# kowallus/mbgc

Measured on AMD Instinct MI355X. Metric: input Gbases/s (compress hot path, -m1: match-finding + stream emission), higher is better.
Workload: dtype u8

## Files before the change

mbgc_amd/csrc/swsem_emit.hip:

```cpp
#include "swsem_device.h"
#include "../../include/mbgc_swsem.h"

namespace swk {

constexpr int EMIT_THREADS = 1024;
constexpr uint8_t MATCH_MARK = 0xA5;
constexpr int MAX_EXTEND_MATCH_LEFT_LENGTH = 1 << 24;

struct EMatch {
    uint64_t posSrc, len, posDest, lp;
};

struct EmitContig {
    uint64_t qoff, n;
    uint64_t matchBase;
    uint64_t lock;
    uint64_t scratchBase;
    uint64_t streamBase[SWSEM_NSTREAMS];
    uint32_t cap;
    uint32_t chunk0;
    int32_t factor;
    uint32_t span0;
    int64_t processed, targetIdx;
};

struct EmitOut {
    uint64_t size[SWSEM_NSTREAMS];
    uint64_t unmatchedChars;
    uint64_t extMatched, extMismatches, totalMatched, removed, nmatches;
};

struct LongCopy { uint8_t *dst; const uint8_t *src; uint64_t len; };
constexpr uint32_t LONG_COPY_CAP = 4096;
constexpr uint32_t LONG_COPY_MIN = 32768;

struct EmitView {
    const uint8_t *ref, *qbuf;
    const Match *matches;
    const uint32_t *matchCount;
    uint64_t pos1, refLength, maxRefLength;
    const uint64_t *loaded; uint32_t nLoaded;
    swsem_emit_params_t p;
    EMatch *em;
    uint64_t *next0;
    uint8_t *removed;
    uint32_t *keepIdx;
    uint32_t *meta;
    uint32_t *corr;
    unsigned long long *pairMask;
    unsigned long long *litBits;
    unsigned long long *metaBad;
    uint32_t *sz;
    uint32_t *ofs;
    uint32_t *chunkCnt;
    const uint32_t *chunkOwner;
    const uint32_t *spanOwner;
    uint32_t ncontigs;
    uint64_t *packBase;
    uint8_t *arena;
    struct LongCopy *longCopies;
    uint32_t *longCount;
    EmitOut *out;
};

constexpr uint32_t META_SKIPOFF = 1, META_HASGAP = 2, META_ISGAP = 4, META_GSTART = 8, META_GMID = 16, META_GEND = 32;

__device__ __forceinline__ bool paired(uint64_t aSrc, uint64_t aDst, uint64_t bSrc, uint64_t bDst) {
    return aSrc + bDst == bSrc + aDst;
}

__device__ __forceinline__ int sym5(uint8_t c) {
    return c == 'A' ? 0 : c == 'C' ? 1 : c == 'G' ? 2 : c == 'T' ? 3 : c == 'N' ? 4 : -1;
}
__device__ __forceinline__ uint8_t mismatch2code(uint8_t actual, uint8_t mismatch) {
    const int a = sym5(actual), b = sym5(mismatch);
    if (actual == mismatch || a < 0 || b < 0) return mismatch;
    const uint32_t rows[5] = {0 | 2u << 3 | 0u << 6 | 1u << 9 | 3u << 12, 1 | 0u << 3 | 2u << 6 | 0u << 9 | 3u << 12,
                              0 | 2u << 3 | 0u << 6 | 1u << 9 | 3u << 12, 1 | 0u << 3 | 2u << 6 | 0u << 9 | 3u << 12,
                              1 | 2u << 3 | 3u << 6 | 0u << 9 | 0u << 12};
    return (uint8_t) ((rows[a] >> (3 * b)) & 7u);
}

__device__ __forceinline__ uint64_t loaded_pos(const EmitView &v, uint64_t pos) {
    const uint64_t span = v.refLength - 1;
    const uint64_t back = v.loaded[v.nLoaded - 1];
    while (pos + span < back) pos += span;
    return pos;
}

template <int NT>
__device__ uint32_t block_scan(uint32_t x, uint32_t *lds, uint32_t *total) {
    const uint32_t lane = threadIdx.x & (WAVE - 1), w = threadIdx.x / WAVE;
    uint32_t inc = x;
    for (int d = 1; d < WAVE; d <<= 1) {
        const uint32_t y = (uint32_t) __shfl_up((int) inc, d);
        if ((int) lane >= d) inc += y;
    }
    __syncthreads();
    if (lane == WAVE - 1) lds[w] = inc;
    __syncthreads();
    if (threadIdx.x == 0) {
        uint32_t run = 0;
        for (int i = 0; i < NT / WAVE; i++) { const uint32_t t = lds[i]; lds[i] = run; run += t; }
        lds[NT / WAVE] = run;
    }
    __syncthreads();
    *total = lds[NT / WAVE];
    return lds[w] + inc - x;
}

constexpr int CH = 256;

__device__ __forceinline__ bool p1_flag(const EmitView &v, const Match *__restrict__ M, int64_t n, int64_t j) {
    if (!v.p.enableExtensionsWithMismatches || j < 1 || j + 1 >= n) return false;
    const Match a = M[j - 1], b = M[j], c = M[j + 1];
    return paired(c.posSrc, c.posDest, a.posSrc, a.posDest) && !paired(b.posSrc, b.posDest, a.posSrc, a.posDest) &&
           b.len < v.p.gapBreakingMatchMinLength;
}

__global__ void __launch_bounds__(CH) k_emit_p1_removed(EmitView v, const EmitContig *__restrict__ cgs, const int *__restrict__ which) {
    __shared__ uint32_t cnt;
    const uint32_t gk = v.chunkOwner[blockIdx.x];
    const EmitContig cg = cgs[gk];
    const uint32_t gx = blockIdx.x - cg.chunk0;
    const int64_t n = v.matchCount[which[gk]];
    if ((int64_t) gx * CH >= n) { if (threadIdx.x == 0) v.chunkCnt[(size_t) blockIdx.x] = 0; return; }
    const int64_t j = (int64_t) gx * CH + threadIdx.x;
    if (threadIdx.x == 0) cnt = 0;
    __syncthreads();
    const Match *M = v.matches + cg.matchBase;
    bool keep = false;
    if (j < n) {
        bool r = false;
// ... 241 lines not shown
                st.claimed |= 1ull << (gf - 1);
                if (lazy) {
                    const int t = k + gf;
                    if (t < WAVE) st.nxA = wl64(nextj, t, st.nxA);
                    else st.nxB = wl64(nextj, t - WAVE, st.nxB);
                }
                if (ext && st.gapEndIdx <= j + gf && gf <= v.p.gapDepthMismatchesEncoding) { st.gapStartIdx = j; st.gapEndIdx = j + gf; }
            }
            st.curClaimed = st.claimed & 1ull;
            st.claimed >>= 1;
            if (WRITE) {
                const bool gs = st.gapStartIdx == j, ge = st.gapEndIdx == j + 1, gm = st.gapStartIdx < j && j + 1 < st.gapEndIdx;
                const bool isGap = gs || gm || ge;
                const uint32_t mw = (skipOffset ? META_SKIPOFF : 0) | (gCnt ? META_HASGAP : 0) | (isGap ? META_ISGAP : 0) |
                                    (gs ? META_GSTART : 0) | (gm ? META_GMID : 0) | (ge ? META_GEND : 0) | (gapByte << 8);
                metaV = wl32(mw, k, metaV);
                corrV = wl32(isGap ? (uint32_t) st.gapStartIdx : (uint32_t) j, k, corrV);
            }
        }
        if (WRITE && lane < cnt) {
            v.meta[cg.scratchBase + jl] = metaV;
            v.corr[cg.scratchBase + jl] = corrV;
        }
        st.nxA = st.nxB;
        st.nxB = 0;
    }
}


__device__ __forceinline__ bool mrec_equal(const MetaRec &a, const MetaRec &b) {
    uint32_t ra, rb;
    __builtin_memcpy(&ra, a.rel, 4); __builtin_memcpy(&rb, b.rel, 4);
    uint64_t d = (a.claimed ^ b.claimed) | (uint64_t) (a.gapStartIdx ^ b.gapStartIdx) | (uint64_t) (a.gapEndIdx ^ b.gapEndIdx) |
                 (uint64_t) (a.flags ^ b.flags) | (uint64_t) (ra ^ rb);
#pragma unroll
    for (int e = 0; e < MNX; e++) d |= a.val[e] ^ b.val[e];
    return d == 0;
}

__device__ __forceinline__ void mrec_store(MetaRec *dst, unsigned long long claimed, bool cur, int gs, int ge, const int (&nxPos)[MNX],
                                           const uint64_t (&nxVal)[MNX], bool overflow, int J) {
    uint32_t r[MNX]; uint64_t x[MNX];
#pragma unroll
    for (int e = 0; e < MNX; e++) { r[e] = nxPos[e] >= J ? (uint32_t) (nxPos[e] - J) : 0xFFu; x[e] = nxPos[e] >= J ? nxVal[e] : 0; }
    auto cx = [&](int a, int b) {
        if (r[a] > r[b]) { const uint32_t t = r[a]; r[a] = r[b]; r[b] = t; const uint64_t u = x[a]; x[a] = x[b]; x[b] = u; }
    };
    cx(0, 1); cx(2, 3); cx(0, 2); cx(1, 3); cx(1, 2);
    MetaRec R;
    R.claimed = claimed; R.gapStartIdx = gs; R.gapEndIdx = ge;
    R.flags = (cur ? MREC_CUR : 0u) | (overflow ? MREC_OVERFLOW : 0u);
#pragma unroll
    for (int e = 0; e < MNX; e++) { R.rel[e] = (uint8_t) r[e]; R.val[e] = x[e]; }
    *dst = R;
}

struct MetaSpan { uint32_t gk; int n, B0; bool live; };
__device__ __forceinline__ MetaSpan meta_span(const EmitView &v, const EmitContig *__restrict__ cgs) {
    MetaSpan sp;
    sp.gk = v.spanOwner[blockIdx.x];
    const EmitOut o = v.out[sp.gk];
    sp.n = (int) o.nmatches;
    sp.B0 = (int) (blockIdx.x - cgs[sp.gk].span0) * MSPAN;
    sp.live = o.unmatchedChars != UINT64_MAX && sp.B0 < sp.n;
    return sp;
}

__global__ void __launch_bounds__(CH) k_emit_meta_regions(EmitView v, const EmitContig *__restrict__ cgs) {
    if (!v.p.lazyDecompressionSupport) return;
    const uint32_t gk = v.chunkOwner[blockIdx.x];
    const EmitContig cg = cgs[gk];
    const uint32_t gx = blockIdx.x - cg.chunk0;
    const EmitOut o = v.out[gk];
    if (o.unmatchedChars == UINT64_MAX) return;
    const uint64_t t = (uint64_t) gx * CH + threadIdx.x;
    if (t >= o.nmatches) return;
    const uint64_t lp = loaded_pos(v, v.em[cg.scratchBase + t].posSrc);
    v.em[cg.scratchBase + t].lp = lp;
    uint32_t lo = 0, hi = v.nLoaded;
    while (lo < hi) { const uint32_t mid = (lo + hi) / 2; if (v.loaded[mid] <= lp) lo = mid + 1; else hi = mid; }
    v.next0[cg.scratchBase + t] = lo == v.nLoaded ? UINT64_MAX : v.loaded[lo];
}

__global__ void __launch_bounds__(MLANES) k_emit_meta_masks(EmitView v, const EmitContig *__restrict__ cgs) {
    __shared__ uint64_t skey[MPAD_SIZE], slp[MPAD_SIZE];
    const MetaSpan sp = meta_span(v, cgs);
    if (!sp.live) return;
    const EmitContig cg = cgs[sp.gk];
    const int n = sp.n, B0 = sp.B0, tid = (int) threadIdx.x;
    const int P1 = B0 + MSPAN < n ? B0 + MSPAN : n;
    const int PK = P1 + WAVE < n ? P1 + WAVE : n;
    const EMatch *E = v.em + cg.scratchBase;
    const bool lazy = v.p.lazyDecompressionSupport != 0;
    const int depth = v.p.gapDepthOffsetEncoding;
    for (int i = tid; i < ((PK - B0 + WAVE - 1) & ~(WAVE - 1)); i += MLANES) {
        const int m = B0 + i;
        bool lit0 = false;
        if (m < PK) {
            const EMatch e = E[m];
            const uint64_t side = e.posSrc > cg.lock ? 1u : (e.posSrc < cg.lock ? 2u : 0u);
            skey[mpad(i)] = ((e.posSrc - e.posDest) << 2) | side;
            slp[mpad(i)] = e.lp;
            const uint64_t nxt = m + 1 < n ? E[m + 1].posDest : cg.n;
            lit0 = nxt - (uint32_t) (e.posDest + e.len) == 0;
        }
        const unsigned long long lb = __ballot(lit0);
        if ((tid & (WAVE - 1)) == 0 && m < P1) v.litBits[(size_t) cg.chunk0 * (CH / WAVE) + (size_t) (m / WAVE)] = lb;
    }
    __syncthreads();
    for (int i = tid; i < P1 - B0; i += MLANES) {
        const int m = B0 + i;
        const int gCnt = n - m - 1 < depth ? n - m - 1 : depth;
        const uint64_t kj = skey[mpad(i)];
        const uint64_t own = lazy ? v.next0[cg.scratchBase + m] : UINT64_MAX;
        unsigned long long pm = 0;
#pragma unroll 8
        for (int g = 1; g <= WAVE; g++) {
            const int x = mpad(g <= gCnt ? i + g : i);
            const bool ok = (g <= gCnt) & (skey[x] == kj) & ((slp[x] < own) | !lazy);
            pm |= (unsigned long long) ok << (g - 1);
        }
        v.pairMask[cg.scratchBase + m] = pm;
    }
}

__global__ void __launch_bounds__(MLANES) k_emit_meta_spec(EmitView v, const EmitContig *__restrict__ cgs, MetaRec *__restrict__ recs, int warm,
                                                          unsigned long long *__restrict__ stats) {
    __shared__ uint64_t spm[MPAD_SIZE], sown[MPAD_SIZE];
    __shared__ unsigned long long slit[MPAD_N / WAVE + 2];
    const MetaSpan sp = meta_span(v, cgs);
    if (!sp.live) return;
    const EmitContig cg = cgs[sp.gk];
    const int n = sp.n, B0 = sp.B0, tid = (int) threadIdx.x;
    const int P0 = B0 >= MWARM ? B0 - MWARM : 0;
    const int P1 = B0 + MSPAN < n ? B0 + MSPAN : n;
    const EMatch *E = v.em + cg.scratchBase;
    const bool lazy = v.p.lazyDecompressionSupport != 0, ext = v.p.enableExtensionsWithMismatches != 0;
    const int depth = v.p.gapDepthOffsetEncoding, depthMism = v.p.gapDepthMismatchesEncoding;
    const int PK = P1 + WAVE < n ? P1 + WAVE : n;
    for (int i = tid; i < PK - P0; i += MLANES) {
        if (P0 + i < P1) spm[mpad(i)] = v.pairMask[cg.scratchBase + P0 + i];
        sown[mpad(i)] = lazy ? v.next0[cg.scratchBase + P0 + i] : 0;
    }
    if (tid < MPAD_N / WAVE + 2) {
        const int w = P0 / WAVE + tid;
        slit[tid] = w * WAVE < P1 ? v.litBits[(size_t) cg.chunk0 * (CH / WAVE) + (size_t) w] : 0;
    }
    __syncthreads();
    const int j0 = B0 + tid * MB;
    const bool active = j0 < n;
    const int j1 = j0 + MB < n ? j0 + MB : n;
    unsigned long long claimed = 0;
    bool cur = false, overflow = false;
    int gs = -1, ge = -1;
    int nxPos[MNX]; uint64_t nxVal[MNX];
#pragma unroll
    for (int e = 0; e < MNX; e++) { nxPos[e] = -1; nxVal[e] = 0; }
    MetaRec *myRecs = recs + ((size_t) cg.chunk0 * (CH / MB) + (size_t) (j0 / MB)) * 2;
    for (int s = 0; s < MWARM + MB; s++) {
        const int j = j0 - MWARM + s;
        if (s == MWARM && active) mrec_store(myRecs, claimed, cur, gs, ge, nxPos, nxVal, overflow, j0);
        if (!active || j < j0 - warm || j < 0 || j >= j1) continue;
        const int i = j - P0;
        if (ext && j == ge) { gs = -1; ge = -1; }
        const bool skipOffset = cur;
        const int gCnt = n - j - 1 < depth ? n - j - 1 : depth;
        const bool rule = !lazy && gs == -1 && ((slit[i / WAVE] >> (i & (WAVE - 1))) & 1);
        const unsigned long long taken = claimed | (rule ? 1ull : 0ull);
        unsigned long long em = spm[mpad(i)] & ~taken;
        uint64_t inherited = 0;
#pragma unroll
        for (int e = 0; e < MNX; e++) if (nxPos[e] == j) { inherited = nxVal[e]; nxPos[e] = -1; }
        uint64_t nextj = 0;
        if (lazy) {
            nextj = sown[mpad(i)];
            if (inherited && inherited != nextj) {
                nextj = inherited;
                atomicAdd(&stats[4], 1ull);
                const EMatch mj = E[j];
                em = 0;
                for (int g = 1; g <= gCnt; g++) {
                    const EMatch c = E[j + g];
                    const bool pw = paired(mj.posSrc, mj.posDest, c.posSrc, c.posDest) &&
                                    ((mj.posSrc > cg.lock && c.posSrc > cg.lock) || (mj.posSrc < cg.lock && c.posSrc < cg.lock));
                    if (pw && c.lp < nextj) em |= 1ull << (g - 1);
                }
                em &= ~taken;
            }
        }
        uint32_t gapByte = 0;
        if (em) {
            const int gf = __builtin_ctzll(em) + 1;
            const unsigned long long below = gf > 1 ? ((1ull << (gf - 1)) - 1) : 0ull;
            gapByte = (uint32_t) (gf - __popcll(taken & below));
            claimed |= 1ull << (gf - 1);
            if (lazy && nextj != sown[mpad(i + gf)]) {
                bool put = false;
#pragma unroll
                for (int e = 0; e < MNX; e++) if (!put && nxPos[e] < 0) { nxPos[e] = j + gf; nxVal[e] = nextj; put = true; }
                overflow |= !put;
            }
            if (ext && ge <= j + gf && gf <= depthMism) { gs = j; ge = j + gf; }
        }
        cur = claimed & 1ull;
        claimed >>= 1;
        if (j >= j0) {
            const bool s0 = gs == j, e0 = ge == j + 1, m0 = gs < j && j + 1 < ge;
            const bool isGap = s0 || m0 || e0;
            const uint32_t mw = (skipOffset ? META_SKIPOFF : 0) | (gCnt ? META_HASGAP : 0) | (isGap ? META_ISGAP : 0) |
                                (s0 ? META_GSTART : 0) | (m0 ? META_GMID : 0) | (e0 ? META_GEND : 0) | (gapByte << 8);
            v.meta[cg.scratchBase + j] = mw;
            v.corr[cg.scratchBase + j] = (uint32_t) (isGap ? gs : j);
        }
    }
    if (active) mrec_store(myRecs + 1, claimed, cur, gs, ge, nxPos, nxVal, overflow, j1);
    if (active && overflow) atomicAdd(&stats[7], 1ull);
}

__global__ void __launch_bounds__(WAVE) k_emit_meta_check(EmitView v, const EmitContig *__restrict__ cgs, const MetaRec *__restrict__ recs,
                                                          unsigned long long *__restrict__ stats) {
    constexpr int CPW = WAVE * MB / CH;
    const uint32_t gk = v.chunkOwner[blockIdx.x];
    const EmitContig cg = cgs[gk];
    const uint32_t gx = blockIdx.x - cg.chunk0;
    if (gx % CPW) return;
    const EmitOut o = v.out[gk];
    if (o.unmatchedChars == UINT64_MAX) return;
    const int64_t n = (int64_t) o.nmatches, nblk = (n + MB - 1) / MB;
    const int64_t b = (int64_t) (gx / CPW) * WAVE + threadIdx.x;
    if (b - (int64_t) threadIdx.x >= nblk) return;
    const MetaRec *R0 = recs + (size_t) cg.chunk0 * (CH / MB) * 2;
    bool bad = false;
    if (b < nblk) {
        const MetaRec S = R0[2 * b], F = R0[2 * b + 1];
        bad = ((S.flags | F.flags) & MREC_OVERFLOW) != 0;
        if (b > 0 && !bad) bad = !mrec_equal(S, R0[2 * b - 1]);
    }
    const unsigned long long mb = __ballot(bad);
    if (threadIdx.x == 0) {
        v.metaBad[cg.chunk0 + gx / CPW] = mb;
        if (mb) atomicAdd(&stats[5], (unsigned long long) __popcll(mb));
    }
}

__device__ __forceinline__ void mrec_expand(const MetaRec &R, MetaRun &st) {
    st.claimed = rfl64(R.claimed); st.curClaimed = (rfl32(R.flags) & MREC_CUR) != 0;
    st.gapStartIdx = (int64_t) rfl64((uint64_t) R.gapStartIdx); st.gapEndIdx = (int64_t) rfl64((uint64_t) R.gapEndIdx);
    st.nxA = 0; st.nxB = 0;
#pragma unroll
    for (int e = 0; e < MNX; e++) {
        const int rel = (int) rfl32(R.rel[e]);
        const uint64_t val = rfl64(R.val[e]);
        if (rel < WAVE) st.nxA = wl64(val, rel, st.nxA);
        else if (rel == WAVE) st.nxB = wl64(val, 0, st.nxB);
    }
}

__global__ void __launch_bounds__(WAVE) k_emit_meta_stitch(EmitView v, const EmitContig *__restrict__ cgs, const MetaRec *__restrict__ recs,
                                                           unsigned long long *__restrict__ stats) {
    __shared__ MetaLds L;
    const EmitContig cg = cgs[blockIdx.x];
    const EmitOut o = v.out[blockIdx.x];
    if (o.unmatchedChars == UINT64_MAX) return;
    const int64_t n = (int64_t) o.nmatches;
    const int lane = (int) threadIdx.x;
    const bool lazy = v.p.lazyDecompressionSupport != 0;
    const int64_t nblk = (n + MB - 1) / MB, ngrp = (n + META_GROUP - 1) / META_GROUP;
    constexpr int BPG = META_GROUP / MB;
    const MetaRec *R0 = recs + (size_t) cg.chunk0 * (CH / MB) * 2;
    MetaRun st;
    st.claimed = 0; st.curClaimed = false; st.gapStartIdx = -1; st.gapEndIdx = -1; st.nxA = 0; st.nxB = 0;
    uint32_t replayed = 0;
    const unsigned long long *BW = v.metaBad + cg.chunk0;
    const int64_t nwords = (nblk + WAVE - 1) / WAVE;
    for (int64_t g = 0; g < ngrp;) {
        const int64_t h = BPG * g;
        int64_t first = nblk;
        {
            const MetaRec S = R0[2 * h], F = R0[2 * h + 1];
// ... 713 lines not shown
```

mbgc_amd/csrc/swsem_runtime_emit.h:

```cpp
namespace {

int end_slot(swsem *h, int si) {
    EmitSlot &E = h->slot[si];
    if (!E.outstanding) return SWSEM_OK;
    HIPCHK(hipSetDevice(h->device));
    { int d = run_phase2b(h, E, false); if (d) return d; }
    HIPCHK(hipEventSynchronize(E.evDone));
    E.outstanding = false;
    const int n = E.emitN;
    E.eout.assign((const EmitOut *) E.pinE.p, (const EmitOut *) E.pinE.p + n);
    uint64_t tot = 0;
    E.hostStreamOff.assign((size_t) n * SWSEM_NSTREAMS, 0);
    for (int k = 0; k < n; k++)
        for (int st = 0; st < SWSEM_NSTREAMS; st++) {
            if (E.eout[k].unmatchedChars == UINT64_MAX) E.eout[k].size[st] = 0;
            E.hostStreamOff[(size_t) k * SWSEM_NSTREAMS + st] = tot;
            tot += E.eout[k].size[st];
        }
    E.packedBytes = tot;
    E.hostStreamsValid = false;
    if (h->emitHostCopy) {
        int r = E.next_host_streams(tot + 1);
        if (r) return r;
        if (tot) HIPCHK(hipMemcpyAsync(E.hostStreams().p, E.dEArena.p, tot, hipMemcpyDeviceToHost, h->s3()));
        HIPCHK(hipStreamSynchronize(h->s3()));
        E.hostStreamsValid = true;
    }
    return SWSEM_OK;
}


int emit_layout(swsem *h, EmitSlot &E, int n, const int *contigIdx, const uint64_t *lockPos, const int *factor,
                const int64_t *processed, const int64_t *targetIdx, uint64_t &rows, uint64_t &arena) {
    E.ecg.assign(n, EmitContig());
    std::vector<int> &which = E.ewhich;
    which.assign(n, 0);
    rows = 0; arena = 0;
    E.chunkOwner.clear(); E.spanOwner.clear();
    for (int k = 0; k < n; k++) {
        const int c = contigIdx ? contigIdx[k] : k;
        if (c < 0 || c >= (int) h->contigs.size()) return fail(SWSEM_EINVAL, "swsem_emit: no contig %d in the batch", c);
        which[k] = c;
        EmitContig &e = E.ecg[k];
        const Contig &cg = h->contigs[c];
        const uint64_t nm = cg.n / (h->minLen ? h->minLen : 1) + 2;
        e.qoff = cg.qoff; e.n = cg.n; e.matchBase = cg.matchBase;
        e.lock = lockPos ? lockPos[k] : UINT64_MAX;
        e.scratchBase = rows;
        e.cap = (uint32_t) (nm + 2);
        rows += e.cap;
        e.chunk0 = (uint32_t) E.chunkOwner.size();
        E.chunkOwner.insert(E.chunkOwner.end(), (e.cap + CH - 1) / CH, (uint32_t) k);
        e.span0 = (uint32_t) E.spanOwner.size();
        E.spanOwner.insert(E.spanOwner.end(), (e.cap + MSPAN - 1) / MSPAN, (uint32_t) k);
        e.factor = factor ? factor[k] : 128;
        e.processed = processed ? processed[k] : 0;
        e.targetIdx = targetIdx ? targetIdx[k] : 0;
        const uint64_t szs[SWSEM_NSTREAMS] = {cg.n + nm + 16, 4 * nm + 16, nm + 16, 14 * nm + 16, nm + 16, cg.n + 2 * nm + 16};
        for (int st = 0; st < SWSEM_NSTREAMS; st++) { e.streamBase[st] = arena; arena += (szs[st] + 15) & ~15ull; }
    }
    return SWSEM_OK;
}

int emit_reserve(swsem *h, EmitSlot &E, int n, uint64_t rows, uint64_t arena, uint64_t nLoaded) {
    h->capN = std::max<uint64_t>(h->capN, (uint64_t) n); h->capRows = std::max(h->capRows, rows); h->capArena = std::max(h->capArena, arena);
    if (nLoaded + 1 > h->capLoaded) h->capLoaded = std::max<uint64_t>(4096, 2 * (nLoaded + 1));
    h->capChunks = std::max<uint64_t>(h->capChunks, E.chunkOwner.size());
    const uint64_t N = h->capN, R = h->capRows, A = h->capArena, Cn = h->capChunks;
    int r;
    if ((r = E.dECg.reserve(N)) || (r = E.dEOut.reserve(N)) || (r = E.dEWhich.reserve(N)) || (r = E.dEM.reserve(R)) ||
        (r = E.dENext0.reserve(R)) || (r = E.dERm.reserve(R)) ||
        (r = E.dEKeep.reserve(R)) || (r = E.dEMeta.reserve(R)) || (r = E.dECorr.reserve(R)) ||
        (r = E.dESz.reserve(R * 6)) || (r = E.dEOfs.reserve(R * 6)) || (r = E.dEArena.reserve(A)) || (r = E.dELoaded.reserve(h->capLoaded)) ||
        (r = E.dEStat.reserve(8)) || (r = E.dELong.reserve(LONG_COPY_CAP)) || (r = E.dELongCount.reserve(4)) || (r = E.dEPm.reserve(R)) ||
        (r = E.dELit.reserve((size_t) Cn * (CH / WAVE))) || (r = E.dEBad.reserve(Cn)) || (r = E.dEOwner.reserve(Cn)) || (r = E.dESpanOwner.reserve(Cn)) ||
        (r = E.dEStates.reserve((size_t) Cn * (CH / MB) * 2)) || (r = E.dEChunk.reserve((size_t) Cn * 6)) ||
        (r = E.dEPack.reserve((size_t) N * SWSEM_NSTREAMS)))
        return r;
    if (!E.statZeroed) { HIPCHK(hipMemsetAsync(E.dEStat.p, 0, 8 * sizeof(unsigned long long), h->stream)); E.statZeroed = true; }
    return SWSEM_OK;
}

int emit_upload_tables(swsem *h, EmitSlot &E, int n, const uint64_t *refExtLoadedPos, uint64_t nLoaded, const swsem_spec_finalize_t *spec) {
    hipStream_t up = h->streamUp;
    int r;
    if (!h->roundTopFresh) HIPCHK(hipEventRecord(h->evRoundTop, h->stream));
    h->roundTopFresh = false;
    HIPCHK(hipStreamWaitEvent(up, h->evRoundTop, 0));
    if ((r = upload(h, E.dEOwner.p, E.chunkOwner.data(), E.chunkOwner.size() * sizeof(uint32_t), up))) return r;
    if ((r = upload(h, E.dESpanOwner.p, E.spanOwner.data(), E.spanOwner.size() * sizeof(uint32_t), up))) return r;
    if ((r = upload(h, E.dECg.p, E.ecg.data(), n * sizeof(EmitContig), up)) || (r = upload(h, E.dEWhich.p, E.ewhich.data(), n * sizeof(int), up))) return r;
    E.eloaded.assign(refExtLoadedPos, refExtLoadedPos + nLoaded);
    if ((r = upload(h, E.dELoaded.p, E.eloaded.data(), nLoaded * sizeof(uint64_t), up))) return r;
    if (spec) {
        if ((r = h->dGate.reserve(4)) || (r = h->dPred.reserve(2 * (size_t) n + 64))) return r;
        if ((r = upload(h, h->dPred.p, spec->predExt, n, up)) || (r = upload(h, h->dPred.p + n, spec->predRC, n, up))) return r;
    }
    return flush_copies(h);
}

EmitView emit_book(swsem *h, EmitSlot &E, int si, const swsem_emit_params_t *p, int n, uint64_t nLoaded) {
    EmitView v;
    v.ref = h->ref; v.qbuf = h->qdev; v.matches = h->dMatches.p; v.matchCount = h->dMatchCount.p;
    v.pos1 = (uint64_t) h->ld.pos1; v.refLength = h->refLength(); v.maxRefLength = h->maxRefLength;
    v.loaded = E.dELoaded.p; v.nLoaded = (uint32_t) nLoaded; v.p = *p;
    v.em = E.dEM.p; v.next0 = E.dENext0.p; v.removed = E.dERm.p; v.keepIdx = E.dEKeep.p;
    v.meta = E.dEMeta.p; v.corr = E.dECorr.p; v.sz = E.dESz.p; v.arena = E.dEArena.p; v.out = E.dEOut.p;
    v.packBase = E.dEPack.p;
    v.pairMask = E.dEPm.p; v.litBits = E.dELit.p; v.metaBad = E.dEBad.p;
    v.longCopies = E.dELong.p; v.longCount = E.dELongCount.p;
    v.ofs = E.dEOfs.p;
    v.chunkCnt = E.dEChunk.p;
    v.chunkOwner = E.dEOwner.p; v.spanOwner = E.dESpanOwner.p;
    v.ncontigs = (uint32_t) n;
    E.v2b = v; E.grid2b = (uint32_t) E.chunkOwner.size(); E.n2b = n;
    E.donePending = true;
    h->latest = si; h->selected = -1;
    E.outstanding = true; E.refGuarded = false; E.emitN = n; E.emitPos1 = (uint64_t) h->ld.pos1; E.qdev = h->qdev; E.params = *p;
    E.emitLaps = h->ld.laps;
    uint64_t lm = UINT64_MAX; bool all = true;
    for (int k = 0; k < n; k++) { if (E.ecg[k].lock == UINT64_MAX) all = false; else lm = std::min(lm, E.ecg[k].lock); }
    E.lockMin = all ? lm : UINT64_MAX;
    E.packedBytes = 0; E.hostStreamsValid = false;
    E.deferred2b = false;
    return v;
}

int spec_plan(swsem *h, const swsem_spec_finalize_t *spec, const uint32_t *gate, bool &planned) {
    h->specMode = true;
    int r = finalize_impl(h, spec->ntargets, spec->ext_dev, spec->ext_len, spec->addSep, spec->sep, spec->lazySeparator, spec->lockPos,
                          spec->loadedAfter, gate, true);
    h->specMode = false;
    planned = r == SWSEM_OK;
    if (r == SWSEM_ESPEC) return SWSEM_OK;
    if (r) return r;
    return prepare_inserts(h, h->streamUp);
}

int emit_pass1(swsem *h, EmitSlot &E, const EmitView &v, int n) {
    const dim3 grid2(E.grid2b);
    int r;
    HIPCHK(hipEventRecord(h->evTables, h->streamUp));
    HIPCHK(hipStreamWaitEvent(h->stream, h->evTables, 0));
    hipStream_t sP = h->stream;
    h->mark(SWSEM_K_EMIT, true, sP);
    k_emit_p1_removed<<<grid2, dim3(CH), 0, sP>>>(v, E.dECg.p, E.dEWhich.p);
    k_emit_p1_scan<<<dim3(n), dim3(CH), 0, sP>>>(v, E.dECg.p, E.dEWhich.p);
    k_emit_p1_compact<<<grid2, dim3(CH), 0, sP>>>(v, E.dECg.p, E.dEWhich.p);
    k_emit_p1_finish<<<dim3(n), dim3(CH), 0, sP>>>(v, E.dECg.p);
    h->mark(SWSEM_K_EMIT, false, sP);
    HIPCHK(hipGetLastError());
    if ((r = queue_counts(h, n * sizeof(EmitOut), sP))) return r;
    if ((r = download(h, h->pin.p + h->pinExtraAt, E.dEOut.p, n * sizeof(EmitOut), sP)) || (r = flush_copies(h))) return r;
    HIPCHK(hipEventRecord(h->evP1, sP));
    return SWSEM_OK;
}

int emit_pairing(swsem *h, EmitSlot &E, const EmitView &v, int n) {
    const dim3 grid2(E.grid2b), spans((uint32_t) E.spanOwner.size());
    const size_t outBytes = n * sizeof(EmitOut);
    int r = E.pinE.reserve(outBytes, std::max<size_t>(2 * outBytes, 1 << 20));
    if (r) return r;
    HIPCHK(hipStreamWaitEvent(h->streamAux, h->evP1, 0));
    h->mark(SWSEM_K_EMIT2, true, h->streamAux);
    k_emit_meta_regions<<<grid2, dim3(CH), 0, h->streamAux>>>(v, E.dECg.p);
    k_emit_meta_masks<<<spans, dim3(MLANES), 0, h->streamAux>>>(v, E.dECg.p);
    k_emit_meta_spec<<<spans, dim3(MLANES), 0, h->streamAux>>>(v, E.dECg.p, E.dEStates.p, h->sw.metaWarm, E.dEStat.p);
    HIPCHK(hipEventRecord(h->evMeta, h->streamAux));
    h->metaPending = true;
    k_emit_meta_check<<<grid2, dim3(WAVE), 0, h->streamAux>>>(v, E.dECg.p, E.dEStates.p, E.dEStat.p);
    k_emit_meta_stitch<<<dim3(n), dim3(WAVE), 0, h->streamAux>>>(v, E.dECg.p, E.dEStates.p, E.dEStat.p);
    h->mark(SWSEM_K_EMIT2, false, h->streamAux);
    HIPCHK(hipEventRecord(E.evMetaDone, h->streamAux));
    HIPCHK(hipGetLastError());
    return SWSEM_OK;
}

int spec_gate(swsem *h, EmitSlot &E, const swsem_spec_finalize_t *spec, uint32_t *gate, int n, bool planned, bool &queued, bool &exchanged) {
    k_spec_verify<<<1, 256, 0, h->stream>>>(E.dEOut.p, E.dECg.p, n, h->dPred.p, h->dPred.p + n, spec->factor, spec->rcFactor, gate);
    if (spec->veto || !planned) HIPCHK(hipMemsetAsync(gate, 0, sizeof(uint32_t), h->stream));
    if (spec->exchange) {
        if (spec->exchange(spec->exchange_ctx, 0, gate, (void *) h->stream)) return fail(SWSEM_EHIP, "speculative finalize: the exchange between the replicas failed");
        exchanged = true;
    }
    if (planned) {
        int r = launch_inserts(h, gate);
        if (r) return r;
        queued = true;
    }
    return SWSEM_OK;
}

bool spec_verdict(swsem *h, const EmitSlot &E, const swsem_spec_finalize_t *spec, int n, bool exchanged) {
    bool ok = !spec->veto;
    for (int k = 0; k < n && ok; k++) {
        const uint64_t un = E.eout[k].unmatchedChars, len = E.ecg[k].n;
        ok = un != UINT64_MAX && (un * (uint64_t) spec->factor > len) == (spec->predExt[k] != 0) &&
             (un * (uint64_t) spec->rcFactor > len) == (spec->predRC[k] != 0);
    }
    if (exchanged) ok = spec->exchange(spec->exchange_ctx, 1, nullptr, (void *) h->stream) == 1 && ok;
    return ok;
}

int emit_begin_impl(swsem *h, const swsem_emit_params_t *p, int n, const int *contigIdx, const uint64_t *lockPos,
                    const int *factor, const int64_t *processed, const int64_t *targetIdx,
                    const uint64_t *refExtLoadedPos, uint64_t nLoaded, const swsem_spec_finalize_t *spec, int *applied) {
    HIPCHK(hipSetDevice(h->device));
    if (applied) *applied = 0;
    if (spec && spec->ntargets <= 0) spec = nullptr;
    const int si = h->latest ^ 1;
    { int e = end_slot(h, si); if (e) return e; }
    EmitSlot &E = h->slot[si];
    if (!h->batchValid) return fail(SWSEM_EINVAL, "swsem_emit: no match results on the handle");
    if (n <= 0) return fail(SWSEM_EINVAL, "swsem_emit: empty request");
    if (p->lazyDecompressionSupport && nLoaded == 0) return fail(SWSEM_EINVAL, "swsem_emit: lazy mode needs refExtLoadedPosArr");
    if (p->gapDepthOffsetEncoding > 64 || p->gapDepthOffsetEncoding < 0)
        return fail(SWSEM_EINVAL, "gapDepthOffsetEncoding %d out of range (MAX_GAP_DEPTH / 2)", p->gapDepthOffsetEncoding);
    int r;
    uint64_t rows, arena;
    if ((r = emit_layout(h, E, n, contigIdx, lockPos, factor, processed, targetIdx, rows, arena)) ||
        (r = emit_reserve(h, E, n, rows, arena, nLoaded)) ||
        (r = emit_upload_tables(h, E, n, refExtLoadedPos, nLoaded, spec)))
        return r;
    const EmitView v = emit_book(h, E, si, p, n, nLoaded);
    const LoaderState snap = h->ld;
    bool planned = false, queued = false, exchanged = false;
    uint32_t *gate = spec ? (spec->gate_dev ? spec->gate_dev : h->dGate.p) : nullptr;
    if (spec && (r = spec_plan(h, spec, gate, planned))) return r;
    const bool needCounts = h->matchCount.size() != h->contigs.size();
    if ((r = emit_pass1(h, E, v, n))) return r;
    if ((r = emit_pairing(h, E, v, n))) return r;
    if (spec) {
        if ((r = spec_gate(h, E, spec, gate, n, planned, queued, exchanged))) return r;
        if (!queued) h->ld = snap;
    }
    E.deferred2b = true; E.waitFin2b = queued;
    if (h->emitHostCopy) { int e = end_slot(h, si ^ 1); if (e) return e; }
    HIPCHK(hipEventSynchronize(h->evP1));
    if (needCounts) take_counts(h);
    E.eout.assign((const EmitOut *) (h->pin.p + h->pinExtraAt), (const EmitOut *) (h->pin.p + h->pinExtraAt) + n);
    if (queued) {
        if (spec_verdict(h, E, spec, n, exchanged)) { if (applied) *applied = 1; }
        else h->ld = snap;
    } else if (exchanged)
        (void) spec->exchange(spec->exchange_ctx, 1, nullptr, (void *) h->stream);
    return SWSEM_OK;
}

}
```

mbgc_amd/csrc/swsem_runtime_state.h:

```cpp
#define SWSEM_ESPEC (-100)

namespace {

thread_local std::string g_err;
int fail(int code, const char *fmt, ...) {
    char buf[512];
    va_list ap;
    va_start(ap, fmt);
    vsnprintf(buf, sizeof buf, fmt, ap);
    va_end(ap);
    g_err = buf;
    return code;
}
#define HIPCHK(x) do { hipError_t e_ = (x); if (e_ != hipSuccess) return fail(SWSEM_EHIP, "%s: %s", #x, hipGetErrorString(e_)); } while (0)

constexpr uint64_t REF_SHIFT = 1;
constexpr int SW_WIDTH_FACTOR = 16;
constexpr uint64_t REF_SLACK = 256;
constexpr uint64_t COPY_WGS = 2048;
constexpr uint32_t EMIT_THIN_MAX = 512;
constexpr uint32_t RB_MIN = 2048 / RBU;
constexpr uint32_t CAND_MAX = 4096;
constexpr uint64_t CAND_BYTES = 128ull << 20;
constexpr int NSTATS = 16;

struct NoCopy {
    NoCopy() = default;
    NoCopy(const NoCopy &) = delete;
    NoCopy &operator=(const NoCopy &) = delete;
};
template <typename T>
struct DevBuf : NoCopy {
    T *p = nullptr;
    size_t cap = 0;
    ~DevBuf() { if (p) (void) hipFree(p); }
    int reserve(size_t n) {
        if (n <= cap) return SWSEM_OK;
        if (p) (void) hipFree(p);
        p = nullptr; cap = 0;
        size_t want = n + n / 8 + 64;
        if (hipMalloc((void **) &p, want * sizeof(T)) != hipSuccess) {
            p = nullptr;
            return fail(SWSEM_ENOMEM, "device allocation of %zu bytes failed", want * sizeof(T));
        }
        cap = want;
        return SWSEM_OK;
    }
};

struct PinBuf : NoCopy {
    uint8_t *p = nullptr;
    size_t cap = 0;
    ~PinBuf() { if (p) (void) hipHostFree(p); }
    int reserve(size_t bytes, size_t want, unsigned flags = hipHostMallocCoherent | hipHostMallocMapped) {
        if (bytes <= cap) return SWSEM_OK;
        if (p) (void) hipHostFree(p);
        p = nullptr; cap = 0;
        if (hipHostMalloc((void **) &p, want, flags) != hipSuccess) {
            p = nullptr;
            return fail(SWSEM_ENOMEM, "cannot pin %zu B of host memory", want);
        }
        cap = want;
        return SWSEM_OK;
    }
};

thread_local bool g_eventsFailed = false;
struct Event : NoCopy {
    hipEvent_t e = nullptr;
    Event() { if (hipEventCreateWithFlags(&e, hipEventDisableTiming) != hipSuccess) { e = nullptr; g_eventsFailed = true; } }
    ~Event() { if (e) (void) hipEventDestroy(e); }
    operator hipEvent_t() const { return e; }
};

struct ProfEvent { hipEvent_t a, b; int fam; };

struct LoaderState {
    int64_t pos1 = REF_SHIFT;
    int laps = 0;
    uint64_t samplingPos = 0, swEnd = 0;
    std::deque<uint64_t> locks;
    uint32_t epoch = 1;
    uint32_t eCur = 0, ePrev = 0;
    int64_t sepEndPos = -1; int sepEndLaps = -1, sepEndVal = -1;
    bool pristine = true;
    uint64_t droppedBytes = 0;

    bool sep_end_done(int sep) const { return pos1 == sepEndPos && laps == sepEndLaps && sep == sepEndVal; }
    void sep_end_set(int64_t at, int sep) { sepEndPos = at; sepEndLaps = laps; sepEndVal = sep; }
    uint64_t refLength(uint64_t maxRefLength) const { return laps ? maxRefLength : (uint64_t) pos1; }
    void wrap_if_at_end(uint64_t maxRefLength) {
        if ((uint64_t) pos1 != maxRefLength || swEnd == maxRefLength) return;
        laps++;
        ePrev = eCur; eCur = epoch;
        pos1 = REF_SHIFT;
        samplingPos = REF_SHIFT;
    }
};

struct Switches {
    bool seqResolve = false;
    bool simt = true;
    uint32_t rbFixed = 0;
    int overlapFixed = -1;
    uint32_t profMask = ~0u;
    int metaWarm = swk::MWARM;
    bool lapTags = true;
    bool streamCalib = true;
    bool streamDebug = false;
    bool debugStats = false;
};
Switches read_switches() {
    Switches s;
    if (const char *e = getenv("SWSEM_RESOLVE")) s.seqResolve = strcmp(e, "seq") == 0;
    if (const char *e = getenv("SWSEM_CHAINS")) s.simt = atoi(e) != 1;
    if (const char *e = getenv("SWSEM_RB")) { int x = atoi(e); if (x >= 1 && x <= 256) s.rbFixed = (uint32_t) x * (1024 / RBU); }
    if (const char *e = getenv("SWSEM_OVERLAP")) { int x = atoi(e); if (x >= 0 && x <= swk::OVERLAP_MAX) s.overlapFixed = x; }
    if (const char *e = getenv("SWSEM_PROF_FAMS")) s.profMask = (uint32_t) strtoul(e, nullptr, 0);
    if (const char *e = getenv("SWSEM_META_WARM")) s.metaWarm = std::min(swk::MWARM, std::max(0, atoi(e)));
    if (const char *e = getenv("SWSEM_LAP_TAGS")) s.lapTags = atoi(e) != 0;
    if (const char *e = getenv("SWSEM_STREAM_CALIB")) s.streamCalib = atoi(e) != 0;
    s.streamDebug = getenv("SWSEM_STREAM_DEBUG") != nullptr;
    s.debugStats = getenv("SWSEM_DEBUG_STATS") != nullptr;
    return s;
}

struct PreparedInserts {
    size_t np = 0, nc = 0, nb = 0, ne = 0;
    bool beside = false;
    uint64_t nSamples = 0, nEdge = 0, copyBlocks = 0;
    const InsertPiece *dPieces = nullptr, *dEdge = nullptr;
    const uint64_t *dFirst = nullptr, *dCFirst = nullptr, *dEFirst = nullptr;
    const CopyPiece *dCopies = nullptr;
    const BytePiece *dBytes = nullptr;
};

struct EmitSlot {
    DevBuf<EmitContig> dECg;
    DevBuf<EmitOut> dEOut;
    DevBuf<int> dEWhich;
    DevBuf<uint32_t> dEOwner, dESpanOwner;
    DevBuf<EMatch> dEM;
    DevBuf<uint64_t> dENext0, dELoaded, dEPack;
    DevBuf<uint8_t> dERm, dEArena;
    DevBuf<uint32_t> dEKeep, dEMeta, dECorr, dESz, dEOfs, dEChunk;
    DevBuf<MetaRec> dEStates;
    DevBuf<unsigned long long> dEStat, dEPm, dELit, dEBad;
    DevBuf<LongCopy> dELong;
    DevBuf<uint32_t> dELongCount;
    bool statZeroed = false;
    std::vector<EmitContig> ecg;
    std::vector<uint32_t> chunkOwner, spanOwner;
    std::vector<int> ewhich;
    std::vector<uint64_t> eloaded;
    std::vector<EmitOut> eout;
    Event evDone;
    Event evMetaDone;
    bool outstanding = false, refGuarded = false;
    bool donePending = false;
    bool deferred2b = false, waitFin2b = false;
    EmitView v2b; uint32_t grid2b = 0; int n2b = 0;
    const uint8_t *qdev = nullptr;
    swsem_emit_params_t params;
    uint64_t emitPos1 = 0;
    uint64_t lockMin = UINT64_MAX;
    int emitLaps = 0;
    int emitN = 0;
    PinBuf pinE;
    PinBuf hostHalf[2];
    int hostAt = 0;
    PinBuf &hostStreams() { return hostHalf[hostAt]; }
    int next_host_streams(size_t n) { hostAt ^= 1; return hostStreams().reserve(n, n + n / 2 + 4096, hipHostMallocDefault); }
    std::vector<uint64_t> hostStreamOff;
    bool hostStreamsValid = false;
    uint64_t packedBytes = 0;
};

}

struct swsem {
    int device = 0;
    hipStream_t stream = nullptr;
    bool ownStream = false;
    Switches sw;
    uint8_t *ref = nullptr;
    ht_entry *ht = nullptr;
    uint8_t *lut = nullptr;
    uint16_t *tags = nullptr;
    bool useTags = true;
    LoaderState ld;
    uint64_t maxRefLength = 0;
    int L = 0, K = 0, k1 = 0, skipMargin = 0, k1ord = 0;
    uint32_t hash_size = 0, mask = 0;
    uint64_t swSize = 0;
    bool circular = true;
    int fpBits = 0;
    uint64_t hostProbes = 0;
    bool deferInserts = false;
    bool specMode = false;
    DevBuf<uint32_t> dGate;
    DevBuf<uint8_t> dPred;
    std::vector<InsertPiece> pendingPieces;
    std::vector<InsertPiece> edgePieces;
    int prioLow = 0, prioHigh = 0;
    Event evLoadFork, evLoadDone;
    std::vector<CopyPiece> pendingCopies;
    std::vector<BytePiece> pendingBytes;
    DevBuf<uint64_t> dTables;
    struct HostTab { PinBuf buf; Event ev; bool pending = false; } hostTables[2];
    int hostTableSel = 0;
    PreparedInserts prep;
    hipStream_t stream2 = nullptr, streamLoad = nullptr, streamUp = nullptr, streamAux = nullptr;
    Event evTables, evRoundTop;
    bool roundTopFresh = false;
    DevBuf<uint8_t> stage;
    DevBuf<Contig> dContigs;
    DevBuf<uint32_t> dMatchCount, dRbContig, dRbOrder;
    std::vector<uint32_t> rbOrderHost, rbOrderKey;
    uint32_t chainsPerWave = 1;
    hipStream_t stream3 = nullptr;
    hipStream_t s3() {
        if (!stream3 && hipStreamCreateWithFlags(&stream3, hipStreamNonBlocking) != hipSuccess) stream3 = stream;
        return stream3;
    }
    Event evMatched;
    std::vector<uint32_t> rbContigHost;
    DevBuf<Match> dMatches;
    DevBuf<Row> dRegions, dReplay;
    DevBuf<BlockRec> dRecs;
    DevBuf<FastRec> dFast;
// ... 107 lines not shown
```

Before: 53.71.

## Fuse emit meta region/mask/spec kernels into a single span kernel

Replaces the three-kernel metadata pipeline (regions, masks, spec) with one k_emit_meta_span kernel. It stages match fields in registers and shared memory, computes loaded positions and pair masks in place, then runs the spec scan without a global pairMask or litBits round trip. The dedicated pairMask and litBits buffers are dropped; the legacy split path now reuses the dEOfs buffer as scratch behind an environment switch. This removes two launches and global traffic, at the cost of higher register and shared-memory pressure, and it relies on dEOfs being large enough to hold the masks.

```diff
diff --git a/mbgc_amd/csrc/swsem_emit.hip b/mbgc_amd/csrc/swsem_emit.hip
--- a/mbgc_amd/csrc/swsem_emit.hip
+++ b/mbgc_amd/csrc/swsem_emit.hip
@@ -47,8 +47,6 @@
     uint32_t *keepIdx;
     uint32_t *meta;
     uint32_t *corr;
-    unsigned long long *pairMask;
-    unsigned long long *litBits;
     unsigned long long *metaBad;
     uint32_t *sz;
     uint32_t *ofs;
@@ -456,7 +454,8 @@
     v.next0[cg.scratchBase + t] = lo == v.nLoaded ? UINT64_MAX : v.loaded[lo];
 }
 
-__global__ void __launch_bounds__(MLANES) k_emit_meta_masks(EmitView v, const EmitContig *__restrict__ cgs) {
+__global__ void __launch_bounds__(MLANES) k_emit_meta_masks(EmitView v, const EmitContig *__restrict__ cgs, unsigned long long *__restrict__ pairMask,
+                                                           unsigned long long *__restrict__ litBits) {
     __shared__ uint64_t skey[MPAD_SIZE], slp[MPAD_SIZE];
     const MetaSpan sp = meta_span(v, cgs);
     if (!sp.live) return;
@@ -479,7 +478,7 @@
             lit0 = nxt - (uint32_t) (e.posDest + e.len) == 0;
         }
         const unsigned long long lb = __ballot(lit0);
-        if ((tid & (WAVE - 1)) == 0 && m < P1) v.litBits[(size_t) cg.chunk0 * (CH / WAVE) + (size_t) (m / WAVE)] = lb;
+        if ((tid & (WAVE - 1)) == 0 && m < P1) litBits[(size_t) cg.chunk0 * (CH / WAVE) + (size_t) (m / WAVE)] = lb;
     }
     __syncthreads();
     for (int i = tid; i < P1 - B0; i += MLANES) {
@@ -494,12 +493,13 @@
             const bool ok = (g <= gCnt) & (skey[x] == kj) & ((slp[x] < own) | !lazy);
             pm |= (unsigned long long) ok << (g - 1);
         }
-        v.pairMask[cg.scratchBase + m] = pm;
+        pairMask[cg.scratchBase + m] = pm;
     }
 }
 
 __global__ void __launch_bounds__(MLANES) k_emit_meta_spec(EmitView v, const EmitContig *__restrict__ cgs, MetaRec *__restrict__ recs, int warm,
-                                                          unsigned long long *__restrict__ stats) {
+                                                          unsigned long long *__restrict__ stats, const unsigned long long *__restrict__ pairMask,
+                                                          const unsigned long long *__restrict__ litBits) {
     __shared__ uint64_t spm[MPAD_SIZE], sown[MPAD_SIZE];
     __shared__ unsigned long long slit[MPAD_N / WAVE + 2];
     const MetaSpan sp = meta_span(v, cgs);
@@ -513,12 +513,12 @@
     const int depth = v.p.gapDepthOffsetEncoding, depthMism = v.p.gapDepthMismatchesEncoding;
     const int PK = P1 + WAVE < n ? P1 + WAVE : n;
     for (int i = tid; i < PK - P0; i += MLANES) {
-        if (P0 + i < P1) spm[mpad(i)] = v.pairMask[cg.scratchBase + P0 + i];
+        if (P0 + i < P1) spm[mpad(i)] = pairMask[cg.scratchBase + P0 + i];
         sown[mpad(i)] = lazy ? v.next0[cg.scratchBase + P0 + i] : 0;
     }
     if (tid < MPAD_N / WAVE + 2) {
         const int w = P0 / WAVE + tid;
-        slit[tid] = w * WAVE < P1 ? v.litBits[(size_t) cg.chunk0 * (CH / WAVE) + (size_t) w] : 0;
+        slit[tid] = w * WAVE < P1 ? litBits[(size_t) cg.chunk0 * (CH / WAVE) + (size_t) w] : 0;
     }
     __syncthreads();
     const int j0 = B0 + tid * MB;
@@ -569,6 +569,164 @@
             gapByte = (uint32_t) (gf - __popcll(taken & below));
             claimed |= 1ull << (gf - 1);
             if (lazy && nextj != sown[mpad(i + gf)]) {
+                bool put = false;
+#pragma unroll
+                for (int e = 0; e < MNX; e++) if (!put && nxPos[e] < 0) { nxPos[e] = j + gf; nxVal[e] = nextj; put = true; }
+                overflow |= !put;
+            }
+            if (ext && ge <= j + gf && gf <= depthMism) { gs = j; ge = j + gf; }
+        }
+        cur = claimed & 1ull;
+        claimed >>= 1;
+        if (j >= j0) {
+            const bool s0 = gs == j, e0 = ge == j + 1, m0 = gs < j && j + 1 < ge;
+            const bool isGap = s0 || m0 || e0;
+            const uint32_t mw = (skipOffset ? META_SKIPOFF : 0) | (gCnt ? META_HASGAP : 0) | (isGap ? META_ISGAP : 0) |
+                                (s0 ? META_GSTART : 0) | (m0 ? META_GMID : 0) | (e0 ? META_GEND : 0) | (gapByte << 8);
+            v.meta[cg.scratchBase + j] = mw;
+            v.corr[cg.scratchBase + j] = (uint32_t) (isGap ? gs : j);
+        }
+    }
+    if (active) mrec_store(myRecs + 1, claimed, cur, gs, ge, nxPos, nxVal, overflow, j1);
+    if (active && overflow) atomicAdd(&stats[7], 1ull);
+}
+
+constexpr int MSTAGE = (MPAD_N + MLANES - 1) / MLANES;
+__global__ void __launch_bounds__(MLANES) k_emit_meta_span(EmitView v, const EmitContig *__restrict__ cgs, MetaRec *__restrict__ recs, int warm,
+                                                          unsigned long long *__restrict__ stats) {
+    __shared__ uint64_t sa[MPAD_SIZE], sb[MPAD_SIZE];
+    const MetaSpan sp = meta_span(v, cgs);
+    if (!sp.live) return;
+    const EmitContig cg = cgs[sp.gk];
+    const int n = sp.n, B0 = sp.B0, tid = (int) threadIdx.x;
+    const int P0 = B0 >= MWARM ? B0 - MWARM : 0;
+    const int P1 = B0 + MSPAN < n ? B0 + MSPAN : n;
+    const int PK = P1 + WAVE < n ? P1 + WAVE : n;
+    const int nStaged = PK - P0, nMasks = P1 - P0;
+    EMatch *E = v.em + cg.scratchBase;
+    const bool lazy = v.p.lazyDecompressionSupport != 0, ext = v.p.enableExtensionsWithMismatches != 0;
+    const int depth = v.p.gapDepthOffsetEncoding, depthMism = v.p.gapDepthMismatchesEncoding;
+    uint64_t rs[MSTAGE], rd[MSTAGE], rl[MSTAGE];
+#pragma unroll
+    for (int it = 0; it < MSTAGE; it++) {
+        const int i = it * MLANES + tid;
+        rs[it] = 0; rd[it] = 0; rl[it] = 0;
+        if (i < nStaged) {
+            rs[it] = E[P0 + i].posSrc; rd[it] = E[P0 + i].posDest;
+            if (!lazy) rl[it] = E[P0 + i].len;
+        }
+    }
+    uint64_t own[MSTAGE];
+    const uint64_t wrapSpan = v.refLength - 1, back = lazy ? v.loaded[v.nLoaded - 1] : 0;
+    uint64_t rlo = 1, rhi = 0;
+#pragma unroll
+    for (int it = 0; it < MSTAGE; it++) {
+        const int i = it * MLANES + tid, m = P0 + i;
+        own[it] = 0;
+        if (it * MLANES >= nStaged) break;
+        const uint64_t ps = rs[it], pd = rd[it];
+        if (lazy) {
+            if (i < nStaged) {
+                uint64_t lp = ps;
+                while (lp + wrapSpan < back) lp += wrapSpan;
+                if (lp < rlo || lp >= rhi) {
+                    uint32_t lo = 0, hi = v.nLoaded;
+                    while (lo < hi) { const uint32_t mid = (lo + hi) / 2; if (v.loaded[mid] <= lp) lo = mid + 1; else hi = mid; }
+                    rlo = lo ? v.loaded[lo - 1] : 0;
+                    rhi = lo == v.nLoaded ? UINT64_MAX : v.loaded[lo];
+                }
+                own[it] = rhi;
+                sb[mpad(i)] = lp;
+                if (m >= B0 && m < P1) { E[m].lp = lp; v.next0[cg.scratchBase + m] = rhi; }
+            }
+        } else {
+            uint64_t nxt = (uint64_t) __shfl_down((long long) pd, 1);
+            if (i < nStaged) {
+                if ((tid & (WAVE - 1)) == WAVE - 1 && m + 1 < n) nxt = E[m + 1].posDest;
+                if (m + 1 >= n) nxt = cg.n;
+                sb[mpad(i)] = nxt - (uint32_t) (pd + rl[it]) == 0;
+            }
+        }
+        if (i < nStaged) {
+            const uint64_t side = ps > cg.lock ? 1u : (ps < cg.lock ? 2u : 0u);
+            sa[mpad(i)] = ((ps - pd) << 2) | side;
+        }
+    }
+    __syncthreads();
+    uint64_t pmk[MSTAGE];
+#pragma unroll
+    for (int it = 0; it < MSTAGE; it++) {
+        const int i = it * MLANES + tid, m = P0 + i;
+        unsigned long long pm = 0;
+        if (i < nMasks) {
+            const int gCnt = n - m - 1 < depth ? n - m - 1 : depth;
+            const uint64_t kj = sa[mpad(i)];
+            const uint64_t mine = lazy ? own[it] : UINT64_MAX;
+#pragma unroll 8
+            for (int g = 1; g <= WAVE; g++) {
+                const int x = mpad(g <= gCnt ? i + g : i);
+                const bool ok = (g <= gCnt) & (sa[x] == kj) & ((sb[x] < mine) | !lazy);
+                pm |= (unsigned long long) ok << (g - 1);
+            }
+        }
+        pmk[it] = pm;
+    }
+    __syncthreads();
+#pragma unroll
+    for (int it = 0; it < MSTAGE; it++) {
+        const int i = it * MLANES + tid;
+        if (i < nMasks) sa[mpad(i)] = pmk[it];
+        if (lazy && i < nStaged) sb[mpad(i)] = own[it];
+    }
+    __syncthreads();
+    const int j0 = B0 + tid * MB;
+    const bool active = j0 < n;
+    const int j1 = j0 + MB < n ? j0 + MB : n;
+    unsigned long long claimed = 0;
+    bool cur = false, overflow = false;
+    int gs = -1, ge = -1;
+    int nxPos[MNX]; uint64_t nxVal[MNX];
+#pragma unroll
+    for (int e = 0; e < MNX; e++) { nxPos[e] = -1; nxVal[e] = 0; }
+    MetaRec *myRecs = recs + ((size_t) cg.chunk0 * (CH / MB) + (size_t) (j0 / MB)) * 2;
+    for (int s = 0; s < MWARM + MB; s++) {
+        const int j = j0 - MWARM + s;
+        if (s == MWARM && active) mrec_store(myRecs, claimed, cur, gs, ge, nxPos, nxVal, overflow, j0);
+        if (!active || j < j0 - warm || j < 0 || j >= j1) continue;
+        const int i = j - P0;
+        if (ext && j == ge) { gs = -1; ge = -1; }
+        const bool skipOffset = cur;
+        const int gCnt = n - j - 1 < depth ? n - j - 1 : depth;
+        const bool rule = !lazy && gs == -1 && (sb[mpad(i)] & 1);
+        const unsigned long long taken = claimed | (rule ? 1ull : 0ull);
+        unsigned long long em = sa[mpad(i)] & ~taken;
+        uint64_t inherited = 0;
+#pragma unroll
+        for (int e = 0; e < MNX; e++) if (nxPos[e] == j) { inherited = nxVal[e]; nxPos[e] = -1; }
+        uint64_t nextj = 0;
+        if (lazy) {
+            nextj = sb[mpad(i)];
+            if (inherited && inherited != nextj) {
+                nextj = inherited;
+                atomicAdd(&stats[4], 1ull);
+                const EMatch mj = E[j];
+                em = 0;
+                for (int g = 1; g <= gCnt; g++) {
+                    const EMatch c = E[j + g];
+                    const bool pw = paired(mj.posSrc, mj.posDest, c.posSrc, c.posDest) &&
+                                    ((mj.posSrc > cg.lock && c.posSrc > cg.lock) || (mj.posSrc < cg.lock && c.posSrc < cg.lock));
+                    if (pw && loaded_pos(v, c.posSrc) < nextj) em |= 1ull << (g - 1);
+                }
+                em &= ~taken;
+            }
+        }
+        uint32_t gapByte = 0;
+        if (em) {
+            const int gf = __builtin_ctzll(em) + 1;
+            const unsigned long long below = gf > 1 ? ((1ull << (gf - 1)) - 1) : 0ull;
+            gapByte = (uint32_t) (gf - __popcll(taken & below));
+            claimed |= 1ull << (gf - 1);
+            if (lazy && nextj != sb[mpad(i + gf)]) {
                 bool put = false;
 #pragma unroll
                 for (int e = 0; e < MNX; e++) if (!put && nxPos[e] < 0) { nxPos[e] = j + gf; nxVal[e] = nextj; put = true; }
diff --git a/mbgc_amd/csrc/swsem_runtime_emit.h b/mbgc_amd/csrc/swsem_runtime_emit.h
--- a/mbgc_amd/csrc/swsem_runtime_emit.h
+++ b/mbgc_amd/csrc/swsem_runtime_emit.h
@@ -72,8 +72,8 @@
         (r = E.dENext0.reserve(R)) || (r = E.dERm.reserve(R)) ||
         (r = E.dEKeep.reserve(R)) || (r = E.dEMeta.reserve(R)) || (r = E.dECorr.reserve(R)) ||
         (r = E.dESz.reserve(R * 6)) || (r = E.dEOfs.reserve(R * 6)) || (r = E.dEArena.reserve(A)) || (r = E.dELoaded.reserve(h->capLoaded)) ||
-        (r = E.dEStat.reserve(8)) || (r = E.dELong.reserve(LONG_COPY_CAP)) || (r = E.dELongCount.reserve(4)) || (r = E.dEPm.reserve(R)) ||
-        (r = E.dELit.reserve((size_t) Cn * (CH / WAVE))) || (r = E.dEBad.reserve(Cn)) || (r = E.dEOwner.reserve(Cn)) || (r = E.dESpanOwner.reserve(Cn)) ||
+        (r = E.dEStat.reserve(8)) || (r = E.dELong.reserve(LONG_COPY_CAP)) || (r = E.dELongCount.reserve(4)) ||
+        (r = E.dEBad.reserve(Cn)) || (r = E.dEOwner.reserve(Cn)) || (r = E.dESpanOwner.reserve(Cn)) ||
         (r = E.dEStates.reserve((size_t) Cn * (CH / MB) * 2)) || (r = E.dEChunk.reserve((size_t) Cn * 6)) ||
         (r = E.dEPack.reserve((size_t) N * SWSEM_NSTREAMS)))
         return r;
@@ -107,7 +107,7 @@
     v.em = E.dEM.p; v.next0 = E.dENext0.p; v.removed = E.dERm.p; v.keepIdx = E.dEKeep.p;
     v.meta = E.dEMeta.p; v.corr = E.dECorr.p; v.sz = E.dESz.p; v.arena = E.dEArena.p; v.out = E.dEOut.p;
     v.packBase = E.dEPack.p;
-    v.pairMask = E.dEPm.p; v.litBits = E.dELit.p; v.metaBad = E.dEBad.p;
+    v.metaBad = E.dEBad.p;
     v.longCopies = E.dELong.p; v.longCount = E.dELongCount.p;
     v.ofs = E.dEOfs.p;
     v.chunkCnt = E.dEChunk.p;
@@ -163,9 +163,14 @@
     if (r) return r;
     HIPCHK(hipStreamWaitEvent(h->streamAux, h->evP1, 0));
     h->mark(SWSEM_K_EMIT2, true, h->streamAux);
-    k_emit_meta_regions<<<grid2, dim3(CH), 0, h->streamAux>>>(v, E.dECg.p);
-    k_emit_meta_masks<<<spans, dim3(MLANES), 0, h->streamAux>>>(v, E.dECg.p);
-    k_emit_meta_spec<<<spans, dim3(MLANES), 0, h->streamAux>>>(v, E.dECg.p, E.dEStates.p, h->sw.metaWarm, E.dEStat.p);
+    if (!h->sw.metaSplit)
+        k_emit_meta_span<<<spans, dim3(MLANES), 0, h->streamAux>>>(v, E.dECg.p, E.dEStates.p, h->sw.metaWarm, E.dEStat.p);
+    else {
+        unsigned long long *pairMask = (unsigned long long *) E.dEOfs.p, *litBits = pairMask + h->capRows;
+        k_emit_meta_regions<<<grid2, dim3(CH), 0, h->streamAux>>>(v, E.dECg.p);
+        k_emit_meta_masks<<<spans, dim3(MLANES), 0, h->streamAux>>>(v, E.dECg.p, pairMask, litBits);
+        k_emit_meta_spec<<<spans, dim3(MLANES), 0, h->streamAux>>>(v, E.dECg.p, E.dEStates.p, h->sw.metaWarm, E.dEStat.p, pairMask, litBits);
+    }
     HIPCHK(hipEventRecord(h->evMeta, h->streamAux));
     h->metaPending = true;
     k_emit_meta_check<<<grid2, dim3(WAVE), 0, h->streamAux>>>(v, E.dECg.p, E.dEStates.p, E.dEStat.p);
diff --git a/mbgc_amd/csrc/swsem_runtime_state.h b/mbgc_amd/csrc/swsem_runtime_state.h
--- a/mbgc_amd/csrc/swsem_runtime_state.h
+++ b/mbgc_amd/csrc/swsem_runtime_state.h
@@ -105,6 +105,7 @@
     int overlapFixed = -1;
     uint32_t profMask = ~0u;
     int metaWarm = swk::MWARM;
+    bool metaSplit = false;
     bool lapTags = true;
     bool streamCalib = true;
     bool streamDebug = false;
@@ -118,6 +119,7 @@
     if (const char *e = getenv("SWSEM_OVERLAP")) { int x = atoi(e); if (x >= 0 && x <= swk::OVERLAP_MAX) s.overlapFixed = x; }
     if (const char *e = getenv("SWSEM_PROF_FAMS")) s.profMask = (uint32_t) strtoul(e, nullptr, 0);
     if (const char *e = getenv("SWSEM_META_WARM")) s.metaWarm = std::min(swk::MWARM, std::max(0, atoi(e)));
+    if (const char *e = getenv("SWSEM_META_SPLIT")) s.metaSplit = atoi(e) != 0;
     if (const char *e = getenv("SWSEM_LAP_TAGS")) s.lapTags = atoi(e) != 0;
     if (const char *e = getenv("SWSEM_STREAM_CALIB")) s.streamCalib = atoi(e) != 0;
     s.streamDebug = getenv("SWSEM_STREAM_DEBUG") != nullptr;
@@ -145,7 +147,7 @@
     DevBuf<uint8_t> dERm, dEArena;
     DevBuf<uint32_t> dEKeep, dEMeta, dECorr, dESz, dEOfs, dEChunk;
     DevBuf<MetaRec> dEStates;
-    DevBuf<unsigned long long> dEStat, dEPm, dELit, dEBad;
+    DevBuf<unsigned long long> dEStat, dEBad;
     DevBuf<LongCopy> dELong;
     DevBuf<uint32_t> dELongCount;
     bool statZeroed = false;
```

After: 53.25. No clear change (-0.9%).
